# pvjosue/CWFA

Hardware: AMD Instinct MI355X
Metric: volumes/sec inverse-pass @512×512×96 fp32; NLL match vs ref (1/2/4/8 GPU) (higher is better)
Workload: dtype f32 (storage, accumulation, wavelets, couplings); convolution products on the bf16 matrix cores from an exact three-way bf16 split of both fp32 operands, six products per fp32 product: fp32-equivalent; plain-fp32-MFMA figure: fp32_mfma; 1 GPU; 512x512x96 volume, 4-scale CWFA (CAT blocks, 64 ch) + LRNN inverse, z=0, batch 1/GPU, random-init weights (BASELINE.json configs[2]); precision=split, parallelism=replicated x1 (independent volumes per GPU, no collective)

## Files before the change

cwfa_amd/_lib.py:

```python
import ctypes as C
import os

_HERE = os.path.dirname(os.path.abspath(__file__))
LIB_PATH = os.path.join(_HERE, "libcwfa_hip.so")

CLAMP = {"NONE": 0, "ATAN": 1, "TANH": 2, "SIGMOID": 3}
ACT = {None: 0, "none": 0, "elu": 1, "prelu": 2, "gelu": 3, "relu": 4}
CHAIN_MAX = 8

c_f32p = C.c_void_p
c_i64p = C.c_void_p
c_f64p = C.c_void_p


class AffineStage(C.Structure):
    _fields_ = [("s_raw", c_f32p), ("t", c_f32p), ("s_bs", C.c_int64), ("t_bs", C.c_int64), ("clamp_kind", C.c_int),
                ("clamp", C.c_float), ("pre_scale", C.c_float), ("t_neg_div_sqrt2", C.c_int), ("perm", c_i64p),
                ("perm_axis", C.c_int), ("gin", C.c_int)]


class Chain(C.Structure):
    _fields_ = [("n_stages", C.c_int), ("stage", AffineStage * CHAIN_MAX), ("src_c", C.c_void_p), ("src_h", C.c_void_p)]


class ChainGrads(C.Structure):
    _fields_ = [("ds", c_f32p * CHAIN_MAX), ("dt", c_f32p * CHAIN_MAX), ("ds_bs", C.c_int64 * CHAIN_MAX),
                ("dt_bs", C.c_int64 * CHAIN_MAX)]


class ConvOpts(C.Structure):
    _fields_ = [("bias", c_f32p), ("act", C.c_int), ("prelu_alpha", c_f32p), ("residual", c_f32p), ("res_bs", C.c_int64),
                ("act2", C.c_int), ("in_scale", c_f32p), ("in_shift", c_f32p), ("in_affine_bs", C.c_int), ("in_add", c_f32p),
                ("in_add_bs", C.c_int64), ("upshuffle2", C.c_int), ("in_blocked8", C.c_int), ("out_blocked8", C.c_int),
                ("in_cat", c_f32p), ("in_cat_bs", C.c_int64), ("in_cat_from", C.c_int), ("in_cat_c1", C.c_int), ("out_stats", c_f64p), ("prelu_per_channel", C.c_int)]


class Couple(C.Structure):
    _fields_ = [("x", c_f32p), ("y", c_f32p), ("x_bs", C.c_int64), ("y_bs", C.c_int64), ("n", C.c_int), ("clamp_kind", C.c_int),
                ("clamp", C.c_float), ("pre_scale", C.c_float), ("rev", C.c_int), ("logdet", c_f64p), ("in_blocked8", C.c_int)]


class EvalAffine(C.Structure):
    _fields_ = [("enabled", C.c_int), ("scale", C.c_float), ("std", C.c_float), ("mean", C.c_float)]


class EvalPost(C.Structure):
    _fields_ = [("normalize", C.c_int), ("threshold", C.c_int), ("norm_sub", C.c_float), ("norm_div", C.c_float),
                ("vol_min", C.c_float), ("lower", C.c_float), ("upper", C.c_float), ("clamp_value", C.c_float)]


EXTREMA_STRIDE = 12
SELECT_WORKSPACE_BYTES = 8448

i, i64, f, d, p = C.c_int, C.c_int64, C.c_float, C.c_double, C.c_void_p
SIGNATURES = {
    "cwfa_version": (i, []),
    "cwfa_last_error": (C.c_char_p, []),
    "cwfa_set_option": (i, [C.c_char_p, i]),
    "cwfa_haar1d_fwd_f32": (i, [p, p, p, i, i, i64, i64, i64, i64, p]),
    "cwfa_haar1d_inv_f32": (i, [p, p, p, i, i, i64, i64, i64, i64, p]),
    "cwfa_haar2d_fwd_f32": (i, [p, p, i, i, i, i, i, f, p]),
    "cwfa_haar2d_inv_f32": (i, [p, p, i, i, i, i, i, f, p]),
    "cwfa_haar3d_fwd_f32": (i, [p, p, i, i, i, i, i, f, i64, p]),
    "cwfa_haar3d_inv_f32": (i, [p, p, i, i, i, i, i, f, i64, p]),
    "cwfa_gather_f32": (i, [p, p, p, i, i, i, i, i, i64, i64, p]),
    "cwfa_affine_f32": (i, [p, p, C.POINTER(AffineStage), i, i, i, i, i, i64, i64, p, p, p]),
    "cwfa_channel_affine_f32": (i, [p, p, p, p, i, p, p, i, i, i64, i64, i64, p]),
# ... 101 lines not shown
```

cwfa_amd/csrc/conv2d.hip:

```cpp
#include "conv_internal.h"

#include <string.h>
#include <type_traits>

namespace {

template <int KS_, int CK_, int MT_, int NT_, int WM_, int WN_, int XV_ = 1>
struct Cfg {
    static constexpr int KS = KS_, CK = CK_, MT = MT_, NT = NT_, WM = WM_, WN = WN_;
    static constexpr int XV = XV_;
    static_assert(XV_ == 1 || (XV_ == 4 && KS_ == 1), "vector staging needs halo-free tiles");
    static constexpr int PAD = KS / 2;
    static constexpr int NTHREADS = 64 * WM * WN;
    static constexpr int CT = 32 * MT * WM;
    static constexpr int TR = NT * WN;
    static constexpr int TC = 32;
    static constexpr int XR = TR + KS - 1;
    static constexpr int XC = TC + KS - 1;
    static constexpr int XS = CK * XR * XC;
    static constexpr int XS_PAD = (XS + 3) & ~3;
    static constexpr int WS = KS * KS * CK * CT;
    static constexpr int XPT = (XS / XV + NTHREADS - 1) / NTHREADS;
    static constexpr int WPT = (WS / 4 + NTHREADS - 1) / NTHREADS;
    static constexpr int BUF = XS_PAD + WS;
// ... 539 lines not shown
            if constexpr (ALLOWED & (1u << EPI_NONE_BLK8)) return launch_epi<C, EPI_NONE_BLK8, PRO>(p, st);
            cwfa_set_error("cwfa_conv2d_f32: out_blocked8 is built for the 1x1 kernels with more than 32 output channels");
            return CWFA_E_SHAPE;
        default: break;
    }
    return launch_epi<C, EPI_GENERIC, PRO>(p, st);
}

template <class C, unsigned ALLOWED, unsigned ALLOWED_PRO>
int launch(const ConvParams& p, int epi, hipStream_t st) {
    if (p.o.in_scale || p.o.in_add) return launch_sel<C, ALLOWED_PRO, true>(p, epi, st);
    return launch_sel<C, ALLOWED, false>(p, epi, st);
}

}
int g_cwfa_split_xcd_map = 1;
int g_cwfa_split_rows16 = 1;
extern int g_cwfa_mip3_ablate;
namespace {

int fill_params(ConvParams& p, const char* name, const float* x, const float* w_packed, float* y, int B, int Cin, int H,
                int W, int Cout, int64_t x_bs, int64_t y_bs, const cwfa_conv_opts* opts) {
    CWFA_REQUIRE(B >= 0 && Cin > 0 && Cout > 0 && H >= 0 && W >= 0, CWFA_E_INVAL, "%s: bad size", name);
    if (B == 0 || H == 0 || W == 0) return 1;
    CWFA_REQUIRE(x && w_packed && y, CWFA_E_INVAL, "%s: null pointer", name);
    CWFA_REQUIRE((int64_t)Cin * H * W < (1ll << 30) && (int64_t)Cout * H * W * (p.o.upshuffle2 ? 1 : 1) < (1ll << 30), CWFA_E_SHAPE, "%s: C*H*W exceeds the 32-bit byte offsets of a tile (2^30 elements per image)", name);
    CWFA_REQUIRE(cwfa_aligned16(w_packed), CWFA_E_ALIGN, "%s: packed weights must be 16-byte aligned", name);
    p.x = x; p.wp = w_packed; p.y = y;
    p.B = B; p.Cin = Cin; p.H = H; p.W = W; p.Cout = Cout;
    p.x_bs = x_bs; p.y_bs = y_bs;
    p.products = g_cwfa_operand == CwfaOperand::split3 ? 6 : 1;
    if (opts) p.o = *opts;
    CWFA_REQUIRE(!(p.o.in_scale && !p.o.in_shift), CWFA_E_INVAL, "%s: in_scale without in_shift", name);
    CWFA_REQUIRE(p.o.act >= 0 && p.o.act <= CWFA_ACT_RELU && p.o.act2 >= 0 && p.o.act2 <= CWFA_ACT_RELU, CWFA_E_INVAL,
                 "%s: bad activation", name);
    CWFA_REQUIRE(!((p.o.act == CWFA_ACT_PRELU || p.o.act2 == CWFA_ACT_PRELU) && !p.o.prelu_alpha), CWFA_E_INVAL,
                 "%s: PReLU without prelu_alpha", name);
    return CWFA_OK;
}

typedef Cfg<1, 16, 2, 4, 4, 2> CS;
constexpr int CS_XB = 3 * 2 * 8 * 32 * 16, CS_WB = 3 * 2 * 256 * 16, CS_BUFB = CS_XB + CS_WB;

__device__ __forceinline__ void split3(float v, unsigned short (&o)[3]) {
    const __bf16 a1 = (__bf16)v;
    const float r1 = v - (float)a1;
    const __bf16 a2 = (__bf16)r1;
    const float r2 = r1 - (float)a2;
    const __bf16 a3 = (__bf16)r2;
    o[0] = __builtin_bit_cast(unsigned short, a1);
    o[1] = __builtin_bit_cast(unsigned short, a2);
    o[2] = __builtin_bit_cast(unsigned short, a3);
}

__device__ __forceinline__ unsigned short f16_bits(float v) { return __builtin_bit_cast(unsigned short, (_Float16)v); }

template <bool F16 = false>
__global__ __launch_bounds__(256) void split_input_kernel(const float* __restrict__ x, uint4* __restrict__ ws, int Cin, int CG2,
                                                          int64_t HW, int64_t x_bs, const float* __restrict__ sc,
                                                          const float* __restrict__ sh, int64_t aff_bs,
                                                          const float* __restrict__ add, int64_t add_bs) {
    const int64_t px = (int64_t)blockIdx.x * 256 + threadIdx.x;
    if (px >= HW) return;
    const int cg = blockIdx.y, b = blockIdx.z;
    unsigned short pc[3][8];
#pragma unroll
// ... 433 lines not shown
```

cwfa_amd/csrc/conv_split3x3.hip:

```cpp
#include "conv_internal.h"

extern int g_cwfa_split_xcd_map;
extern int g_cwfa_split_rows16;

namespace {

constexpr int TR = 8, TC = 32;

template <int KS, int RPW = 4>
struct XG {
    static constexpr int TRW = 2 * RPW, NT = 2 * RPW;
    static constexpr int PAD = KS / 2, XR = TRW + 2 * PAD, XC = TC + 2 * PAD, NTAP = KS * KS;
    static constexpr int EPK = XR * XC;
    static constexpr int KHB = KS == 7 ? 8512 : RPW == 8 ? 9792 : 5440;
    static constexpr int XPB = 2 * KHB;
    static constexpr int XB = 3 * XPB;
    static constexpr bool SPECIAL = KS == 3 && RPW == 4;
    static constexpr int NEK = SPECIAL ? 2 : 3;
    static_assert(EPK * 16 <= KHB && KHB % 256 == 64 && 2 * EPK <= 512 * NEK, "staging entry map");
    static_assert(!SPECIAL || (EPK > 256 && EPK <= 384), "3x3 staging entry map");
    static_assert(KS == 3 || RPW == 4, "7x7: 8-row tiles");
};

template <int MPW, int KS = 3, int RPW = 4, int WM = 4>
// ... 55 lines not shown

    constexpr int NEK = G::NEK;
    int ekh[NEK], eidx[NEK];
    bool fin[NEK];
    unsigned fo[NEK];
    if constexpr (SPECIAL) {
        ekh[0] = wave >> 2; eidx[0] = tid & 255; fin[0] = true;
        ekh[1] = (wave >> 1) & 1; eidx[1] = 256 + (tid & 127); fin[1] = wave < 4 && eidx[1] < EPK;
    } else {
#pragma unroll
        for (int k = 0; k < NEK; ++k) {
            const int e = tid + 512 * k;
            ekh[k] = e >= EPK;
            eidx[k] = e - ekh[k] * EPK;
            fin[k] = e < 2 * EPK;
        }
    }
    bool fok[NEK];
#pragma unroll
    for (int k = 0; k < NEK; ++k) {
        const int r = eidx[k] / XC, c = eidx[k] % XC;
        const int gr = row0 + r - PAD, gc = col0 + c - PAD;
        fok[k] = fin[k] && gr >= 0 && gr < p.H && gc >= 0 && gc < p.W;
        fo[k] = !fok[k] ? OOB : p.o.in_blocked8 ? (unsigned)((gr * p.W + gc) * 32) : (unsigned)((gr * p.W + gc) * 4);
        if constexpr (!SPECIAL) fo[k] = !fok[k] ? OOB : fo[k] + (unsigned)(ekh[k] * 8) * (unsigned)plane;
    }
    const int xbytes = p.Cin * plane;
    const auto rx = CWFA_RSRC(p.x + (int64_t)b * p.x_bs, xbytes);
    const auto ra = CWFA_RSRC(ADD ? p.o.in_add + (int64_t)b * p.o.in_add_bs : p.x, ADD ? xbytes : 0);
    const bool has_aff = p.o.in_scale != nullptr;
    typedef const float __attribute__((address_space(4))) cfloat;
    cfloat* sc = has_aff ? (cfloat*)(p.o.in_scale + (int64_t)b * p.o.in_affine_bs) : nullptr;
    cfloat* sh = has_aff ? (cfloat*)(p.o.in_shift + (int64_t)b * p.o.in_affine_bs) : nullptr;

    auto load_entry = [&](auto kc, float (&xv)[8], float (&av)[8], int chunk) {
        constexpr int k = decltype(kc)::value;
        const int ch0 = chunk * 16 + (SPECIAL ? ekh[k] * 8 : 0);
        if (KS == 3 && !ADD && p.o.in_blocked8) {
            const f32x4 lo4 = __builtin_bit_cast(f32x4, __builtin_amdgcn_raw_buffer_load_b128(rx, fo[k], ch0 * plane, 0));
            const f32x4 hi4 = __builtin_bit_cast(f32x4, __builtin_amdgcn_raw_buffer_load_b128(rx, fo[k], ch0 * plane + 16, 0));
#pragma unroll
            for (int j = 0; j < 4; ++j) {
                xv[j] = lo4[j];
                xv[4 + j] = hi4[j];
            }
            return;
        }
#pragma unroll
        for (int j = 0; j < 8; ++j) xv[j] = __builtin_bit_cast(float, __builtin_amdgcn_raw_buffer_load_b32(rx, fo[k], (ch0 + j) * plane, 0));
        if constexpr (ADD) {
#pragma unroll
            for (int j = 0; j < 8; ++j) av[j] = __builtin_bit_cast(float, __builtin_amdgcn_raw_buffer_load_b32(ra, fo[k], (ch0 + j) * plane, 0));
        }
    };
    auto store_entry = [&](auto kc, const float (&xv)[8], const float (&av)[8], int chunk, int buf) {
        constexpr int k = decltype(kc)::value;
        if (SPECIAL && k == 1 && !fin[1]) return;
        const int ch0 = chunk * 16 + ekh[k] * 8;
        bf16x8 pc[3];
        float scv[8], shv[8];
        if (has_aff) {
#pragma unroll
            for (int j = 0; j < 8; ++j) {
                const int ch = ch0 + j < p.Cin ? ch0 + j : p.Cin - 1;
                scv[j] = ch0 + j < p.Cin ? sc[ch] : 0.f;
                shv[j] = ch0 + j < p.Cin ? sh[ch] : 0.f;
            }
        }
#pragma unroll
        for (int j = 0; j < 8; ++j) {
            float v = xv[j];
            if (has_aff) v = fok[k] ? v * scv[j] + shv[j] : 0.f;
            if constexpr (ADD) v += av[j];
            __bf16 a1, a2 = (__bf16)0.f, a3 = (__bf16)0.f;
            cwfa_split3<SIX, F16>(v, a1, a2, a3);
            pc[0][j] = a1; pc[1][j] = a2; pc[2][j] = a3;
        }
        char* dst = lds + buf * XB + ekh[k] * KHB + eidx[k] * 16;
        if (SPECIAL || fin[k]) {
#pragma unroll
            for (int q = 0; q < NQ; ++q) *reinterpret_cast<bf16x8*>(dst + q * XPB) = pc[q];
        }
    };

    constexpr int NPC = (SIX ? WSL : WSL / 3) / 1024;
    const int64_t wtile = (int64_t)ct * p.nsteps * WSL;
    const char* wbase = reinterpret_cast<const char*>(p.wp) + wtile;
    const auto rw = CWFA_RSRC(wbase, p.nsteps * WSL);
    auto dma_w = [&](int slice, int slot) {
        cwfa_static_for<(NPC + 7) / 8>([&](auto ic_) {
            constexpr int i = decltype(ic_)::value;
            const int piece = i * 8 + wave;
            if (piece < NPC) {
                char* dst = lds + OFF_W + slot * WSL + piece * 1024;
                __builtin_amdgcn_raw_ptr_buffer_load_lds(rw, (lds_ptr)dst, 16, (unsigned)(lane * 16), slice * WSL + piece * 1024, 0, 0);
            }
        });
    };

    const int alane = OFF_W + (g * CT + wm * MPW * 16 + c16) * 16;
    const int blane = (g & 1) * KHB + (wn * RW * XC + c16) * 16;
    const bool sel = (g >> 1) != 0;

    f32x4 acc[MPW][NT];
#pragma unroll
    for (int mt = 0; mt < MPW; ++mt)
// ... 438 lines not shown

extern "C" int64_t cwfa_conv3x3_split_packed_bytes(int Cout, int Cin) {
    if (Cout <= 0 || Cin <= 0) return -1;
    const int ct = ct_of(Cout);
    return (int64_t)((Cout + ct - 1) / ct) * nsteps_of(Cin) * 3 * 4 * ct * 16;
}

extern "C" int cwfa_conv3x3_split_pack_f32(const float* w, void* packed, int Cout, int Cin, void* stream) {
    CWFA_REQUIRE(w && packed, CWFA_E_INVAL, "cwfa_conv3x3_split_pack_f32: null pointer");
    CWFA_REQUIRE(Cout > 0 && Cin > 0, CWFA_E_SHAPE, "cwfa_conv3x3_split_pack_f32: bad shape");
    CWFA_REQUIRE(cwfa_aligned16(packed), CWFA_E_ALIGN, "cwfa_conv3x3_split_pack_f32: packed image must be 16-byte aligned");
    pack_bank(w, packed, Cout, Cin, ct_of(Cout), 9, (hipStream_t)stream);
    CWFA_LAUNCH_CHECK("cwfa_conv3x3_split_pack_f32");
    return CWFA_OK;
}

extern "C" int cwfa_conv3x3_split_f32(const float* x, const void* w_packed, float* y, int B, int Cin, int H, int W, int Cout,
                                      int64_t x_bs, int64_t y_bs, const cwfa_conv_opts* opts, void* stream) {
    CWFA_REQUIRE(B >= 0 && Cin > 0 && Cout > 0 && H >= 0 && W >= 0, CWFA_E_INVAL, "cwfa_conv3x3_split_f32: bad size");
    if (B == 0 || H == 0 || W == 0) return CWFA_OK;
    CWFA_REQUIRE(x && w_packed && y, CWFA_E_INVAL, "cwfa_conv3x3_split_f32: null pointer");
    CWFA_REQUIRE(cwfa_aligned16(w_packed), CWFA_E_ALIGN, "cwfa_conv3x3_split_f32: packed weights must be 16-byte aligned");
    SParams p{};
    p.x = x; p.wp = w_packed; p.y = y;
    p.B = B; p.Cin = Cin; p.H = H; p.W = W; p.Cout = Cout; p.x_bs = x_bs; p.y_bs = y_bs;
    if (opts) p.o = *opts;
    CWFA_REQUIRE(!p.o.upshuffle2 && !p.o.in_cat, CWFA_E_SHAPE, "cwfa_conv3x3_split_f32: upshuffle2 / in_cat are 1x1 features");
    CWFA_REQUIRE(!p.o.in_blocked8 || (Cin % 8 == 0 && cwfa_aligned16(x) && (x_bs & 3) == 0 && !p.o.in_add), CWFA_E_ALIGN,
                 "cwfa_conv3x3_split_f32: blocked input needs Cin %% 8 == 0, 16-byte alignment and no added tensor");
    CWFA_REQUIRE(!p.o.out_blocked8 || (Cout % 8 == 0 && cwfa_aligned16(y) && (y_bs & 3) == 0 && !p.o.residual && p.o.act2 == CWFA_ACT_NONE &&
                                       (p.o.act == CWFA_ACT_NONE || p.o.act == CWFA_ACT_PRELU)),
                 CWFA_E_ALIGN, "cwfa_conv3x3_split_f32: blocked output needs Cout %% 8 == 0, 16-byte alignment and a bias / PReLU epilogue");
    CWFA_REQUIRE(!(p.o.in_scale && !p.o.in_shift), CWFA_E_INVAL, "cwfa_conv3x3_split_f32: in_scale without in_shift");
    CWFA_REQUIRE(!p.o.out_stats || (!p.o.out_blocked8 && !p.o.residual && p.o.act2 == CWFA_ACT_NONE &&
                                    (p.o.act == CWFA_ACT_NONE || p.o.act == CWFA_ACT_PRELU)),
                 CWFA_E_INVAL, "cwfa_conv3x3_split_f32: out_stats needs an NCHW output and a bias / PReLU epilogue");
    CWFA_REQUIRE(!((p.o.out_stats || p.o.out_blocked8) && p.o.in_add && p.o.act == CWFA_ACT_NONE), CWFA_E_INVAL,
                 "cwfa_conv3x3_split_f32: out_stats / out_blocked8 with in_add need a PReLU epilogue");
    CWFA_REQUIRE(p.o.act >= 0 && p.o.act <= CWFA_ACT_RELU && p.o.act2 >= 0 && p.o.act2 <= CWFA_ACT_RELU, CWFA_E_INVAL,
                 "cwfa_conv3x3_split_f32: bad activation");
    CWFA_REQUIRE(!((p.o.act == CWFA_ACT_PRELU || p.o.act2 == CWFA_ACT_PRELU) && !p.o.prelu_alpha), CWFA_E_INVAL,
                 "cwfa_conv3x3_split_f32: PReLU without prelu_alpha");
    p.nchunks = (Cin + 15) / 16;
    p.nsteps = nsteps_of(Cin);
    p.nrun = p.nsteps - ((p.nchunks & 1) ? 4 : 0);
    p.tiles_x = (W + TC - 1) / TC;
    const int mpw = mpw_of(Cout);
    CWFA_REQUIRE((int64_t)(Cin + 64) * H * W * 4 < (1ll << 31) && (int64_t)(Cout + 64 * mpw) * H * W * 4 < (1ll << 31) &&
                     (int64_t)(p.nsteps + 2) * 3 * 4 * 64 * mpw * 16 < (1ll << 31), CWFA_E_SHAPE,
                 "cwfa_conv3x3_split_f32: one sample's input / output / one cout tile's weights must stay below 2 GiB");
    CWFA_REQUIRE((int64_t)p.tiles_x * ((H + TR - 1) / TR) < (1ll << 31) && B <= 65535, CWFA_E_SHAPE, "cwfa_conv3x3_split_f32: grid too large");
    hipStream_t st = (hipStream_t)stream;
    const int wm = wm_of(Cout);
    if (wm != 4) {
        CWFA_REQUIRE(!p.o.in_scale && !p.o.in_add && !p.o.out_blocked8, CWFA_E_INVAL,
                     "cwfa_conv3x3_split_f32: banks with <= 48 or 65 .. 96 outputs take no load-side prologue and write NCHW");
        const bool plain = !p.o.residual && p.o.act2 == CWFA_ACT_NONE;
        const int epi = plain && p.o.act == CWFA_ACT_NONE ? 0 : plain && p.o.act == CWFA_ACT_PRELU ? 1 : 2;
#define CWFA_NARROW(M, W_)                                                                                                                   \
    do {                                                                                                                                     \
        if (epi == 0) return launch<M, false, CWFA_ACT_NONE, 3, 8, W_>(p, st);                                                               \
        if (epi == 1) return launch<M, false, CWFA_ACT_PRELU, 3, 8, W_>(p, st);                                                              \
        return launch<M, false, EPI_RUNTIME, 3, 8, W_>(p, st);                                                                               \
    } while (0)
        if (mpw == 3 && wm == 2) CWFA_NARROW(3, 2);
        if (mpw == 3) CWFA_NARROW(3, 1);
        if (mpw == 2) CWFA_NARROW(2, 1);
        CWFA_NARROW(1, 1);
#undef CWFA_NARROW
    }
    if (mpw == 4) return launch_epi<4>(p, st);
    if (mpw == 2) return launch_epi<2>(p, st);
    if (g_cwfa_split_rows16 && H > 8 && !p.o.in_scale && !p.o.in_add && !p.o.residual && p.o.act == CWFA_ACT_NONE && p.o.act2 == CWFA_ACT_NONE)
        return launch<2, false, CWFA_ACT_NONE, 3, 8, 2>(p, st);
    if (g_cwfa_split_rows16 && H > 8 && !p.o.in_scale && !p.o.in_add && !p.o.out_stats && !p.o.out_blocked8)
        return launch<2, false, EPI_RUNTIME, 3, 8, 2>(p, st);
    return launch_epi<1>(p, st);
}

extern "C" int64_t cwfa_conv7x7_split_packed_bytes(int Cout, int Cin) {
    if (Cout <= 0 || Cout > 64 || Cin <= 0) return -1;
    return (int64_t)nsteps_of(Cin, 49) * 3 * 4 * 64 * 16;
}

extern "C" int cwfa_conv7x7_split_pack_f32(const float* w, void* packed, int Cout, int Cin, void* stream) {
    CWFA_REQUIRE(w && packed, CWFA_E_INVAL, "cwfa_conv7x7_split_pack_f32: null pointer");
    CWFA_REQUIRE(Cout > 0 && Cout <= 64 && Cin > 0, CWFA_E_SHAPE, "cwfa_conv7x7_split_pack_f32: 1 <= Cout <= 64");
    CWFA_REQUIRE(cwfa_aligned16(packed), CWFA_E_ALIGN, "cwfa_conv7x7_split_pack_f32: packed image must be 16-byte aligned");
    pack_bank(w, packed, Cout, Cin, 64, 49, (hipStream_t)stream);
    CWFA_LAUNCH_CHECK("cwfa_conv7x7_split_pack_f32");
    return CWFA_OK;
}

extern "C" int cwfa_conv7x7_split_f32(const float* x, const void* w_packed, float* y, int B, int Cin, int H, int W, int Cout,
                                      int64_t x_bs, int64_t y_bs, const cwfa_conv_opts* opts, void* stream) {
    CWFA_REQUIRE(B >= 0 && Cin > 0 && Cout > 0 && Cout <= 64 && H >= 0 && W >= 0, CWFA_E_INVAL, "cwfa_conv7x7_split_f32: bad size (Cout <= 64)");
    if (B == 0 || H == 0 || W == 0) return CWFA_OK;
    CWFA_REQUIRE(x && w_packed && y, CWFA_E_INVAL, "cwfa_conv7x7_split_f32: null pointer");
    CWFA_REQUIRE(cwfa_aligned16(w_packed), CWFA_E_ALIGN, "cwfa_conv7x7_split_f32: packed weights must be 16-byte aligned");
    SParams p{};
    p.x = x; p.wp = w_packed; p.y = y;
    p.B = B; p.Cin = Cin; p.H = H; p.W = W; p.Cout = Cout; p.x_bs = x_bs; p.y_bs = y_bs;
    if (opts) p.o = *opts;
    CWFA_REQUIRE(!p.o.upshuffle2 && !p.o.in_cat && !p.o.in_scale && !p.o.in_add && !p.o.in_blocked8 && !p.o.out_blocked8 && !p.o.residual && !p.o.out_stats &&
                     p.o.act == CWFA_ACT_NONE && p.o.act2 == CWFA_ACT_NONE,
                 CWFA_E_INVAL, "cwfa_conv7x7_split_f32: bias-only epilogue, no load-side prologue, NCHW maps");
    p.nchunks = (Cin + 15) / 16;
    p.nsteps = nsteps_of(Cin, 49);
    p.nrun = p.nsteps;
    p.tiles_x = (W + TC - 1) / TC;
    CWFA_REQUIRE((int64_t)(Cin + 64) * H * W * 4 < (1ll << 31) && (int64_t)(Cout + 64) * H * W * 4 < (1ll << 31), CWFA_E_SHAPE,
                 "cwfa_conv7x7_split_f32: one sample's input / output must stay below 2 GiB");
    CWFA_REQUIRE((int64_t)p.tiles_x * ((H + TR - 1) / TR) < (1ll << 31) && B <= 65535, CWFA_E_SHAPE, "cwfa_conv7x7_split_f32: grid too large");
    hipStream_t st = (hipStream_t)stream;
    return launch<2, false, CWFA_ACT_NONE, 7, 4, 2>(p, st);
}
```

cwfa_amd/ops.py:

```python
import ctypes as C

import torch

from . import _lib
from ._lib import AffineStage, Chain, ConvOpts, check

__all__ = ["haar1d", "haar2d", "gather", "affine", "channel_affine", "chain_inv", "chain_fwd", "pack_conv_weight",
           "conv2d", "conv2d_wgrad", "elu_bwd", "set_precision", "gelu_add", "gelu_bwd", "layernorm_bwd", "attention_bwd", "plane_affine", "bn_bwd_stats", "bn_act_bwd", "maxpool2_bwd", "chain_bwd", "chain_inv_bwd", "prelu_bwd", "conv3d_1k1_backward", "pack_1x1_panel", "pack_split_layer_weight", "subnet_layer", "conv3d_1k1", "channel_stats", "bn_fold", "bn_running_update", "maxpool", "sample_stats", "layernorm_apply",
           "attention_combine", "scale_channels", "axpby", "stage"]


def _stream():
    return C.c_void_p(torch.cuda.current_stream().cuda_stream)


def _p(t):
    return None if t is None else C.c_void_p(t.data_ptr())


def _dev(t, name="tensor"):
    if not torch.is_tensor(t):
        raise TypeError(f"{name}: expected a torch.Tensor, got {type(t)}")
    if not t.is_cuda:
        raise RuntimeError(f"{name}: cwfa_amd runs on MI355X only -- got a {t.device} tensor (no CPU fallback exists)")
# ... 343 lines not shown
        return PackedConv(packed, cout, cin, ks, transposed, w._version, w.data_ptr(), split=True)
    if not direct and SPLIT_7X7 and _split_bf16 >= 2 and ks == 7 and cout <= 64 and cin >= 32:
        packed = torch.empty(L.cwfa_conv7x7_split_packed_bytes(cout, cin), dtype=torch.uint8, device=w.device)
        check(L.cwfa_conv7x7_split_pack_f32(_p(w), _p(packed), cout, cin, _stream()), "conv7x7_split_pack")
        return PackedConv(packed, cout, cin, ks, transposed, w._version, w.data_ptr(), split=True)
    n = L.cwfa_conv2d_packed_floats(cout, cin, ks)
    if n <= 0:
        raise ValueError(f"unsupported filter bank {tuple(w.shape)}")
    packed = torch.empty(n, dtype=torch.float32, device=w.device)
    check(L.cwfa_conv2d_pack_f32(_p(w), _p(packed), cout, cin, ks, int(transposed), _stream()), "conv2d_pack")
    return PackedConv(packed, cout, cin, ks, transposed, w._version, w.data_ptr())


def pack_conv_weight_cat(w, c1):
    w = _dev(w, "weight").detach()
    cout, cin, ks, kw = w.shape
    if ks != 1 or kw != 1 or cout > 64 or not (0 < c1 < cin):
        raise ValueError(f"pack_conv_weight_cat: a 1x1 bank with <= 64 outputs and 0 < c1 < Cin is needed, got {tuple(w.shape)}, c1 = {c1}")
    start = (c1 + 15) // 16 * 16
    wz = torch.zeros((cout, start + cin - c1, 1, 1), dtype=torch.float32, device=w.device)
    wz[:, :c1] = w[:, :c1]
    wz[:, start:] = w[:, c1:]
    pc = pack_conv_weight(wz)
    pc.version, pc.src_ptr = w._version, w.data_ptr()
    pc.cat_c1, pc.cat_from = c1, start
    return pc


def conv_writes_stats(pc, act=None, residual=None, act2=None, out_blocked=False, in_add=False):
    return bool(pc.split and pc.ks == 3 and act in (None, "prelu") and residual is None and act2 is None and not out_blocked
                and not (in_add and act is None))


def conv2d(x, pc, bias=None, act=None, prelu_alpha=None, residual=None, act2=None, in_scale=None, in_shift=None,
           in_add=None, out=None, in_blocked=False, out_blocked=False, cat=None, out_stats=None):
    L = _lib.lib()
    x, xbs = planes(x, "x")
    B, Cin, H, W = x.shape
    o = ConvOpts()
    keep = [x]
    if cat is not None:
        cat, cbs = planes(cat, "cat")
        c1 = getattr(pc, "cat_c1", None)
        if c1 is None or Cin != c1 or tuple(cat.shape) != (B, pc.cin - pc.cat_from, H, W) or in_scale is not None or in_add is not None:
            raise ValueError("conv2d: `cat` needs a bank from pack_conv_weight_cat for exactly these two inputs, and no load-side prologue")
        o.in_cat, o.in_cat_bs, o.in_cat_from, o.in_cat_c1 = cat.data_ptr(), cbs, pc.cat_from, c1
        keep.append(cat)
        Cin = pc.cin
    if Cin != pc.cin:
        raise ValueError(f"conv2d: input has {Cin} channels, filter bank expects {pc.cin}")
    up = bool(pc.transposed)
    oshape = (B, pc.cout // 4, 2 * H, 2 * W) if up else (B, pc.cout, H, W)
    if out is None:
        out = torch.empty(oshape, dtype=torch.float32, device=x.device)
        ybs = oshape[1] * oshape[2] * oshape[3]
    else:
        if tuple(out.shape) != oshape:
            raise ValueError(f"conv2d: out has shape {tuple(out.shape)}, expected {oshape}")
        out_c, ybs = planes(out, "out")
        if out_c.data_ptr() != out.data_ptr():
            raise ValueError("conv2d: `out` must have contiguous planes")
    if bias is not None:
        o.bias = _dev(bias, "bias").data_ptr()
    o.act, o.act2 = _lib.ACT[act], _lib.ACT[act2]
    if prelu_alpha is not None:
        prelu_alpha = _dev(prelu_alpha, "prelu_alpha")
        o.prelu_alpha = prelu_alpha.data_ptr()
        if prelu_alpha.numel() != 1:
            if prelu_alpha.numel() != pc.cout or not prelu_alpha.is_contiguous() or not (pc.split and pc.ks == 3):
                raise ValueError("conv2d: per-channel PReLU slopes need [Cout] contiguous values and the split-bf16 3x3 kernel")
            o.prelu_per_channel = 1
    elif "prelu" in (act, act2):
        raise ValueError("conv2d: PReLU needs prelu_alpha")
    if residual is not None:
        residual, rbs = planes(residual, "residual")
        if tuple(residual.shape) != oshape:
            raise ValueError(f"conv2d: residual {tuple(residual.shape)} != output {oshape}")
        o.residual, o.res_bs = residual.data_ptr(), rbs
        keep.append(residual)
    if in_scale is not None:
        o.in_scale, o.in_shift = _dev(in_scale).data_ptr(), _dev(in_shift).data_ptr()
        if in_scale.numel() not in (Cin, B * Cin) or in_shift.numel() != in_scale.numel():
            raise ValueError("conv2d: in_scale / in_shift must be [Cin] or [B,Cin]")
        o.in_affine_bs = Cin if (in_scale.numel() == B * Cin and B > 1) else 0
    if in_add is not None:
        in_add, abs_ = planes(in_add, "in_add")
        if tuple(in_add.shape) != tuple(x.shape):
            raise ValueError("conv2d: in_add shape mismatch")
        o.in_add, o.in_add_bs = in_add.data_ptr(), abs_
        keep.append(in_add)
    o.upshuffle2 = int(up)
    if in_blocked:
        if not (pc.split and pc.ks == 3):
            raise ValueError("conv2d: channel-blocked input is read by the split-bf16 3x3 kernel only")
        o.in_blocked8 = 1
    if out_blocked:
        ok3 = (pc.split and pc.ks == 3 and pc.cout % 8 == 0 and residual is None and act2 is None and act in (None, "prelu")
               and not split3x3_narrow(pc.cout) and not (in_add is not None and act is None))
        ok1 = not pc.split and pc.ks == 1 and pc.cout >= 33 and pc.cout % 8 == 0 and not up
        if not (ok3 or ok1):
            raise ValueError("conv2d: channel-blocked output is written by the split-bf16 3x3 kernel (bias / PReLU) and by the "
                             "direct 1x1 kernel with 40..64 output channels only")
        o.out_blocked8 = 1
    if out_stats is not None:
        if not conv_writes_stats(pc, act, residual, act2, out_blocked, in_add is not None):
            raise ValueError("conv2d: out_stats needs the split-bf16 3x3 kernel with an NCHW output and a bias / PReLU epilogue")
        if out_stats.dtype != torch.float64 or out_stats.numel() != 2 * pc.cout or not out_stats.is_cuda:
            raise ValueError("conv2d: out_stats must be a float64 [2*Cout] tensor on the HIP device")
        o.out_stats = out_stats.data_ptr()
    rec = conv_event_sink
    if rec is not None:
        key = (pc.ks, Cin, pc.cout, H, W, B, "%s|%s|%s|%s|%s" % ("pro" if (in_scale is not None or in_add is not None) else "",
                                                                 act or "", "res" if residual is not None else "", act2 or "",
                                                                 ("up" if up else "") + ("+split" if pc.split else "")),
               in_add is not None)
        if rec.want(key):
            e0, e1 = torch.cuda.Event(enable_timing=True), torch.cuda.Event(enable_timing=True)
            e0.record()
    if pc.split and pc.ks == 7:
        if act or act2 or residual is not None or in_scale is not None or in_add is not None:
            raise ValueError("conv2d: the split-bf16 7x7 kernel has a bias-only epilogue and no load-side prologue")
        check(L.cwfa_conv7x7_split_f32(_p(x), _p(pc.packed), _p(out), B, Cin, H, W, pc.cout, xbs, ybs, C.byref(o), _stream()),
              "conv7x7_split")
# ... 58 lines not shown
def conv3x3_couple(u, pc_bias, x, out, clamp_kind, clamp, pre_scale, rev, logdet=None, in_blocked=False):
    L = _lib.lib()
    pc, br = pc_bias
    u, ubs = planes(u, "u")
    B, Cin, H, W = u.shape
    n = pc.cout // 2
    if Cin != pc.cin:
        raise ValueError(f"conv3x3_couple: input has {Cin} channels, filter bank expects {pc.cin}")
    x2, xbs = planes(x, "x")
    o2, obs = planes(out, "out")
    if tuple(x.shape) != (B, n, H, W) or tuple(out.shape) != (B, n, H, W) or o2.data_ptr() != out.data_ptr():
        raise ValueError("conv3x3_couple: x / out must be [B,n,H,W] views with contiguous planes")
    cp = _lib.Couple()
    cp.x, cp.y, cp.x_bs, cp.y_bs, cp.n = x2.data_ptr(), out.data_ptr(), xbs, obs, n
    cp.clamp_kind, cp.clamp, cp.pre_scale, cp.rev = _lib.CLAMP[clamp_kind], float(clamp), float(pre_scale), int(bool(rev))
    if logdet is not None:
        cp.logdet = logdet.data_ptr()
    cp.in_blocked8 = int(bool(in_blocked))
    rec = conv_event_sink
    if rec is not None:
        key = (3, Cin, pc.cout, H, W, B, "||||couple+split", False)
        if rec.want(key):
            e0, e1 = torch.cuda.Event(enable_timing=True), torch.cuda.Event(enable_timing=True)
            e0.record()
    check(L.cwfa_conv3x3_split_couple_f32(_p(u), _p(pc.packed), _p(br), B, Cin, H, W, ubs, C.byref(cp), _stream()),
          "conv3x3_split_couple")
    if rec is not None and rec.want(key):
        e1.record()
        rec.add(key, e0, e1)
    return out


BLOCKED_MAPS = True
SPLIT_7X7 = True
VIRTUAL_CAT = True
COUPLE_EPILOGUE = True


def couple_fused():
    return COUPLE_EPILOGUE and _split_bf16 >= 2


def split3x3_narrow(cout):
    return cout <= 48 or 64 < cout <= 96


SPLIT_3X3_MIN_COUT = 1
SPLIT_3X3_NARROW_MAX = 16
conv_event_sink = None


def pack_1x1_panel(w):
    L = _lib.lib()
    w = _dev(w, "weight").detach().contiguous()
    if tuple(w.shape) != (64, 64, 1, 1):
        raise ValueError("pack_1x1_panel: the fused layer kernel is specialised for 64 channels")
    panel = torch.empty(4096, dtype=torch.float32, device=w.device)
    check(L.cwfa_subnet_pack1x1_f32(_p(w), _p(panel), _stream()), "subnet_pack1x1")
    return PackedConv(panel, 64, 64, 1, False, w._version, w.data_ptr())


def pack_split_layer_weight(w3, w1):
    L = _lib.lib()
    w3 = _dev(w3, "weight").detach().contiguous()
    w1 = _dev(w1, "weight").detach().contiguous()
    if tuple(w3.shape) != (64, 64, 3, 3) or tuple(w1.shape) != (64, 64, 1, 1):
# ... 709 lines not shown
```

cwfa_amd/unet.py:

```python
import torch
from torch import nn

from . import ops
from .amp import amp_entry

__all__ = ["UNet", "UNetConvBlock", "UNetUpBlock"]


_MATERIALIZE_UP = False
_MATERIALIZE = True


class _Packed:

    def __init__(self):
        self._c = {}

    def get(self, conv, transposed=False):
        w = conv.weight
        pc = self._c.get(id(conv))
        if pc is None or pc.version != w._version or pc.src_ptr != w.data_ptr() or pc.epoch != ops.pack_epoch():
            pc = self._c[id(conv)] = ops.pack_conv_weight(w, transposed=transposed)
        return pc

# ... 81 lines not shown
                 activation=nn.LeakyReLU):
        super().__init__()
        if stride != 1 or kernel_size != 3 or not padding:
            raise NotImplementedError("cwfa_amd UNetConvBlock: 3x3, stride 1, padded convolutions only")
        block = [nn.Conv2d(in_size, out_size, kernel_size=kernel_size, stride=stride, padding=int(padding), bias=use_bias),
                 activation()]
        if batch_norm:
            block.append(nn.BatchNorm2d(out_size))
        block += [nn.Conv2d(out_size, out_size, kernel_size=kernel_size, stride=1, padding=int(padding), bias=use_bias),
                  activation()]
        if batch_norm:
            block.append(nn.BatchNorm2d(out_size))
        self.block = nn.Sequential(*block)
        self.batch_norm = batch_norm
        self._packed = _Packed()

    def _layers(self):
        mods = list(self.block)
        step = 3 if self.batch_norm else 2
        return [(mods[i], mods[i + 1], mods[i + 2] if self.batch_norm else None) for i in (0, step)]

    @staticmethod
    def _act(a):
        if isinstance(a, nn.PReLU):
            if a.weight.numel() != 1:
                raise NotImplementedError("per-channel PReLU")
            return "prelu", a.weight
        if isinstance(a, nn.ELU):
            return "elu", None
        if isinstance(a, nn.ReLU):
            return "relu", None
        raise NotImplementedError(f"activation {type(a).__name__} has no HIP epilogue")

    def run(self, x, in_affine=None, in_add=None, out_mask=None):
        aff = in_affine
        layers = self._layers()
        packs = [self._packed.get(conv) for conv, _, _ in layers]
        for li, (conv, act, bn) in enumerate(layers):
            kind, alpha = self._act(act)
            sc, sh = aff if aff is not None else (None, None)
            add = in_add if li == 0 else None
            if (_MATERIALIZE and ops._split_bf16 < 2 and (sc is not None or add is not None)
                    and (x.shape[2] * x.shape[3]) % 4 == 0):
                x = ops.plane_affine(x, sc, sh, add=add)
                sc = sh = add = None
            st = None
            if (STATS_IN_EPILOGUE and bn is not None and _bn_batch_stats(bn)
                    and ops.conv_writes_stats(packs[li], kind, in_add=add is not None)):
                st = _bn_stats_buffer(bn, x.device)
            x = ops.conv2d(x, packs[li], bias=conv.bias, act=kind, prelu_alpha=alpha, in_scale=sc,
                           in_shift=sh, in_add=add, out_stats=st)
            last = li == len(layers) - 1
            m = out_mask if last else None
            if bn is not None:
                aff = _bn_affine(bn, x, m, stats=st)
            elif m is not None:
                aff = _drop_affine(x.shape[1], m)
            else:
                aff = None
        return x, aff

    @amp_entry
    def forward(self, x):
        y, aff = self.run(x)
        if aff is None:
            return y
        return ops.channel_affine(y, aff[0], aff[1])


class UNetUpBlock(nn.Module):

    def __init__(self, in_size, out_size, up_mode, padding, batch_norm, use_bias=False, skip_conn=True,
                 activation=nn.Softplus):
        super().__init__()
        self.skip_conn = skip_conn
        if up_mode != 'upconv':
            raise NotImplementedError("cwfa_amd UNetUpBlock: up_mode='upconv' only (what the LRNN uses, networks.py:532)")
        self.up = nn.ConvTranspose2d(in_size, out_size, kernel_size=2, stride=2, bias=use_bias)
        in_size = out_size if not skip_conn else in_size // 2
        self.conv_block = UNetConvBlock(in_size, out_size, padding, batch_norm, use_bias=use_bias, activation=activation)
        self._packed = _Packed()

    @staticmethod
    def center_crop(layer, target_size):
        _, _, h, w = layer.size()
        dy, dx = (h - target_size[0]) // 2, (w - target_size[1]) // 2
        return layer[:, :, dy:(dy + target_size[0]), dx:(dx + target_size[1])]

    def run(self, x, bridge, in_affine=None, out_mask=None):
        sc, sh = in_affine if in_affine is not None else (None, None)
        if _MATERIALIZE_UP and ops._split_bf16 < 1 and sc is not None and (x.shape[2] * x.shape[3]) % 4 == 0:
            x = ops.plane_affine(x, sc, sh)
            sc = sh = None
        up = ops.conv2d(x, self._packed.get(self.up, transposed=True), bias=self.up.bias, in_scale=sc, in_shift=sh)
        add = self.center_crop(bridge, up.shape[2:]) if self.skip_conn else None
        return self.conv_block.run(up, in_add=add, out_mask=out_mask)

    @amp_entry
    def forward(self, x, bridge):
        y, aff = self.run(x, bridge)
        return y if aff is None else ops.channel_affine(y, aff[0], aff[1])


class UNet(nn.Module):

    def __init__(self, in_channels=1, n_classes=2, depth=5, wf=6, padding=True, batch_norm=True, up_mode='upsample',
                 drop_out=0, use_bias=False, skip_conn=False, activation=nn.PReLU):
        super().__init__()
        assert up_mode in ('upconv', 'upsample')
        self.padding, self.depth, self.skip_conn, self.drop_out = padding, depth, skip_conn, drop_out
        prev = in_channels
        self.down_path = nn.ModuleList()
        for i in range(depth):
            self.down_path.append(UNetConvBlock(prev, 2 ** (wf + i), padding, batch_norm, use_bias=use_bias,
                                                activation=activation))
            prev = 2 ** (wf + i)
        self.up_path = nn.ModuleList()
        for i in reversed(range(depth - 1)):
            self.up_path.append(UNetUpBlock(prev, 2 ** (wf + i), up_mode, padding, batch_norm, use_bias=use_bias,
                                            skip_conn=skip_conn, activation=activation))
            prev = 2 ** (wf + i)
        self.last = nn.Sequential(nn.Conv2d(prev, n_classes, kernel_size=1, bias=use_bias), activation())
        self._packed = _Packed()

    @amp_entry
    def forward(self, x, store_activations=False, in_affine=None):
        if store_activations:
            raise NotImplementedError("store_activations is a debugging aid of the reference, not on the hot path")
        B, dev = x.shape[0], x.device
        skips, aff = [], in_affine
        n_draw = 0
        if self.drop_out:
            n_draw = B * (sum(d.block[0].out_channels for d in list(self.down_path)[:-1]) +
                          sum(u.conv_block.block[0].out_channels for u in self.up_path))
        pool = _DrawPool(n_draw, dev)
        for i, down in enumerate(self.down_path):
            x, aff = down.run(x, in_affine=aff)
            if i != len(self.down_path) - 1:
                sc, sh = aff if aff is not None else (None, None)
                x, full = ops.maxpool(x, x.shape[-1] // 2, x.shape[-1] // 2, sc, sh, want_full=True)
                skips.append(full)
                m = _drop(self.drop_out, B, x.shape[1], dev, pool)
                aff = _drop_affine(x.shape[1], m) if m is not None else None
        for i, up in enumerate(self.up_path):
            m = _drop(self.drop_out, B, up.conv_block.block[0].out_channels, dev, pool)
            x, aff = up.run(x, skips[-i - 1], in_affine=aff, out_mask=m)
        kind, alpha = UNetConvBlock._act(self.last[1])
        sc, sh = aff if aff is not None else (None, None)
        return ops.conv2d(x, self._packed.get(self.last[0]), bias=self.last[0].bias, act=kind, prelu_alpha=alpha,
                          in_scale=sc, in_shift=sh)
```

include/cwfa_hip.h:

```cpp
#ifndef CWFA_HIP_H
#define CWFA_HIP_H

#include <stdint.h>

#ifdef __cplusplus
extern "C" {
#endif

#define CWFA_VERSION 100

enum {
    CWFA_OK = 0,
    CWFA_E_INVAL = -1,
    CWFA_E_SHAPE = -2,
    CWFA_E_ALIGN = -3,
    CWFA_E_HIP = -4
};

enum { CWFA_CLAMP_NONE = 0, CWFA_CLAMP_ATAN = 1, CWFA_CLAMP_TANH = 2, CWFA_CLAMP_SIGMOID = 3 };

enum { CWFA_ACT_NONE = 0, CWFA_ACT_ELU = 1, CWFA_ACT_PRELU = 2, CWFA_ACT_GELU = 3, CWFA_ACT_RELU = 4 };

int cwfa_version(void);
const char* cwfa_last_error(void);
// ... 51 lines not shown
} cwfa_chain;

int cwfa_chain_inv_f32(const float* z, const float* low, float* x, const cwfa_chain* ch, int B, int C, int H, int W,
                       int64_t z_bs, int64_t low_bs, int64_t x_bs, double* logdet, void* stream);

int cwfa_chain_fwd_f32(const float* x, float* low, float* z, const cwfa_chain* ch, const int64_t* final_perm,
                       int B, int C, int H, int W, int64_t x_bs, int64_t low_bs, int64_t z_bs,
                       double* logdet, double* sumsq, void* stream);


int64_t cwfa_conv2d_packed_floats(int Cout, int Cin, int ks);
int cwfa_conv2d_pack_f32(const float* w, float* packed, int Cout, int Cin, int ks, int transposed, void* stream);

typedef struct {
    const float* bias;
    int act;
    const float* prelu_alpha;
    const float* residual;
    int64_t res_bs;
    int act2;
    const float* in_scale;
    const float* in_shift;
    int in_affine_bs;
    const float* in_add;
    int64_t in_add_bs;
    int upshuffle2;
    int in_blocked8;
    int out_blocked8;
    const float* in_cat;
    int64_t in_cat_bs;
    int in_cat_from, in_cat_c1;
    double* out_stats;
    int prelu_per_channel;
} cwfa_conv_opts;

int cwfa_conv2d_f32(const float* x, const float* w_packed, float* y, int B, int Cin, int H, int W, int Cout, int ks,
                    int64_t x_bs, int64_t y_bs, const cwfa_conv_opts* opts, void* stream);

int cwfa_subnet_pack1x1_f32(const float* w, float* panel, void* stream);
int cwfa_subnet_layer_f32(const float* x, const float* w3_packed, const float* b3, const float* w1_panel, const float* b1,
                          float* y, int B, int H, int W, int64_t x_bs, int64_t y_bs, void* stream);
int cwfa_subnet_layer_tape_f32(const float* x, const float* w3_packed, const float* b3, const float* w1_panel, const float* b1,
                               float* y, float* hidden, int B, int H, int W, int64_t x_bs, int64_t y_bs, int64_t hidden_bs,
                               void* stream);

int cwfa_conv3d_1k1_f32(const float* x, const float* w1, const float* b1, const float* alpha, const float* w2,
                        const float* b2, float* y, int B, int D, int H, int W, int K, void* stream);
int cwfa_conv3d_1k1_split_f32(const float* x, const float* w1, const float* b1, const float* alpha, const float* w2,
                              const float* b2, float* y, int B, int D, int H, int W, int K, void* stream);


int cwfa_channel_stats_f32(const float* x, double* stats, int B, int C, int64_t HW, int64_t x_bs, void* stream);
int cwfa_bn_fold_f32(const double* stats, double count, const float* running_mean, const float* running_var,
                     const float* weight, const float* bias, float eps, const float* mask_bc, int B, float* scale,
                     float* shift, int C, void* stream);
int cwfa_bn_finish_f32(double* stats, double count, float* running_mean, float* running_var, long long* num_batches_tracked,
                       float momentum, int update_running, const float* weight, const float* bias, float eps, const float* mask_bc,
                       const float* mask_u, float drop_p, float keep_scale, int B, float* scale, float* shift, int C, int zero_stats,
                       void* stream);
int cwfa_bn_running_update_f32(const double* stats, double count, float momentum, float* running_mean, float* running_var,
                               long long* num_batches_tracked, int C, void* stream);
int cwfa_maxpool_f32(const float* x, float* y, float* full, const float* scale, const float* shift, int B, int C,
                     int H, int W, int Ho, int Wo, void* stream);
int cwfa_sample_stats_f32(const float* x, double* stats, int B, int64_t CHW, void* stream);
int cwfa_layernorm_apply_f32(const float* x, const double* stats, const float* w, const float* b, float eps,
                             float* y, int B, int64_t CHW, void* stream);
// ... 134 lines not shown
```

Before: 52.44 volumes/s.

## Defer UNet skip-connection batchnorm affine into split 3x3 conv add-load

Instead of having maxpool write out a fully normalized copy of each down-path activation for the skip connection, the UNet keeps the raw pre-affine map plus its scale/shift. The first 3x3 split-bf16 conv of the matching up block then applies that per-channel affine to the in_add operand while loading it. The aim is to drop one full-resolution activation write and its later reread per skip level. In exchange, the conv staging path does extra per-channel scalar loads and FMAs, the raw skip tensors stay alive longer, and narrow tilings fall back to a separate channel_affine pass.

Result: no change. 52.51 volumes/s (median of 6 runs) (+0.1%).

```diff
diff --git a/cwfa_amd/_lib.py b/cwfa_amd/_lib.py
--- a/cwfa_amd/_lib.py
+++ b/cwfa_amd/_lib.py
@@ -32,7 +32,8 @@
     _fields_ = [("bias", c_f32p), ("act", C.c_int), ("prelu_alpha", c_f32p), ("residual", c_f32p), ("res_bs", C.c_int64),
                 ("act2", C.c_int), ("in_scale", c_f32p), ("in_shift", c_f32p), ("in_affine_bs", C.c_int), ("in_add", c_f32p),
                 ("in_add_bs", C.c_int64), ("upshuffle2", C.c_int), ("in_blocked8", C.c_int), ("out_blocked8", C.c_int),
-                ("in_cat", c_f32p), ("in_cat_bs", C.c_int64), ("in_cat_from", C.c_int), ("in_cat_c1", C.c_int), ("out_stats", c_f64p), ("prelu_per_channel", C.c_int)]
+                ("in_cat", c_f32p), ("in_cat_bs", C.c_int64), ("in_cat_from", C.c_int), ("in_cat_c1", C.c_int), ("out_stats", c_f64p), ("prelu_per_channel", C.c_int),
+                ("in_add_scale", c_f32p), ("in_add_shift", c_f32p), ("in_add_affine_bs", C.c_int)]
 
 
 class Couple(C.Structure):
diff --git a/cwfa_amd/csrc/conv2d.hip b/cwfa_amd/csrc/conv2d.hip
--- a/cwfa_amd/csrc/conv2d.hip
+++ b/cwfa_amd/csrc/conv2d.hip
@@ -595,6 +595,7 @@
     p.products = g_cwfa_operand == CwfaOperand::split3 ? 6 : 1;
     if (opts) p.o = *opts;
     CWFA_REQUIRE(!(p.o.in_scale && !p.o.in_shift), CWFA_E_INVAL, "%s: in_scale without in_shift", name);
+    CWFA_REQUIRE(!p.o.in_add_scale && !p.o.in_add_shift, CWFA_E_INVAL, "%s: in_add_scale / in_add_shift are features of cwfa_conv3x3_split_f32", name);
     CWFA_REQUIRE(p.o.act >= 0 && p.o.act <= CWFA_ACT_RELU && p.o.act2 >= 0 && p.o.act2 <= CWFA_ACT_RELU, CWFA_E_INVAL,
                  "%s: bad activation", name);
     CWFA_REQUIRE(!((p.o.act == CWFA_ACT_PRELU || p.o.act2 == CWFA_ACT_PRELU) && !p.o.prelu_alpha), CWFA_E_INVAL,
diff --git a/cwfa_amd/csrc/conv_split3x3.hip b/cwfa_amd/csrc/conv_split3x3.hip
--- a/cwfa_amd/csrc/conv_split3x3.hip
+++ b/cwfa_amd/csrc/conv_split3x3.hip
@@ -111,6 +111,7 @@
     typedef const float __attribute__((address_space(4))) cfloat;
     cfloat* sc = has_aff ? (cfloat*)(p.o.in_scale + (int64_t)b * p.o.in_affine_bs) : nullptr;
     cfloat* sh = has_aff ? (cfloat*)(p.o.in_shift + (int64_t)b * p.o.in_affine_bs) : nullptr;
+    const bool has_aaf = ADD && p.o.in_add_scale != nullptr;
 
     auto load_entry = [&](auto kc, float (&xv)[8], float (&av)[8], int chunk) {
         constexpr int k = decltype(kc)::value;
@@ -137,6 +138,25 @@
         if (SPECIAL && k == 1 && !fin[1]) return;
         const int ch0 = chunk * 16 + ekh[k] * 8;
         bf16x8 pc[3];
+        float adv[8];
+        if constexpr (ADD) {
+#pragma unroll
+            for (int j = 0; j < 8; ++j) adv[j] = av[j];
+            if (has_aaf) {
+                cfloat* asc = (cfloat*)(p.o.in_add_scale + (int64_t)b * p.o.in_add_affine_bs);
+                cfloat* ash = (cfloat*)(p.o.in_add_shift + (int64_t)b * p.o.in_add_affine_bs);
+                float tsc[8], tsh[8];
+#pragma unroll
+                for (int j = 0; j < 8; ++j) {
+                    const int ch = ch0 + j < p.Cin ? ch0 + j : p.Cin - 1;
+                    tsc[j] = ch0 + j < p.Cin ? asc[ch] : 0.f;
+                    tsh[j] = ch0 + j < p.Cin ? ash[ch] : 0.f;
+                }
+#pragma unroll
+                for (int j = 0; j < 8; ++j) adv[j] = fok[k] ? adv[j] * tsc[j] + tsh[j] : 0.f;
+                CWFA_FENCE();
+            }
+        }
         float scv[8], shv[8];
         if (has_aff) {
 #pragma unroll
@@ -150,7 +170,7 @@
         for (int j = 0; j < 8; ++j) {
             float v = xv[j];
             if (has_aff) v = fok[k] ? v * scv[j] + shv[j] : 0.f;
-            if constexpr (ADD) v += av[j];
+            if constexpr (ADD) v += adv[j];
             __bf16 a1, a2 = (__bf16)0.f, a3 = (__bf16)0.f;
             cwfa_split3<SIX, F16>(v, a1, a2, a3);
             pc[0][j] = a1; pc[1][j] = a2; pc[2][j] = a3;
@@ -655,6 +675,8 @@
                                        (p.o.act == CWFA_ACT_NONE || p.o.act == CWFA_ACT_PRELU)),
                  CWFA_E_ALIGN, "cwfa_conv3x3_split_f32: blocked output needs Cout %% 8 == 0, 16-byte alignment and a bias / PReLU epilogue");
     CWFA_REQUIRE(!(p.o.in_scale && !p.o.in_shift), CWFA_E_INVAL, "cwfa_conv3x3_split_f32: in_scale without in_shift");
+    CWFA_REQUIRE(!p.o.in_add_scale == !p.o.in_add_shift && !(p.o.in_add_scale && !p.o.in_add), CWFA_E_INVAL,
+                 "cwfa_conv3x3_split_f32: in_add_scale / in_add_shift come together and need in_add");
     CWFA_REQUIRE(!p.o.out_stats || (!p.o.out_blocked8 && !p.o.residual && p.o.act2 == CWFA_ACT_NONE &&
                                     (p.o.act == CWFA_ACT_NONE || p.o.act == CWFA_ACT_PRELU)),
                  CWFA_E_INVAL, "cwfa_conv3x3_split_f32: out_stats needs an NCHW output and a bias / PReLU epilogue");
@@ -676,7 +698,7 @@
     hipStream_t st = (hipStream_t)stream;
     const int wm = wm_of(Cout);
     if (wm != 4) {
-        CWFA_REQUIRE(!p.o.in_scale && !p.o.in_add && !p.o.out_blocked8, CWFA_E_INVAL,
+        CWFA_REQUIRE(!p.o.in_scale && !p.o.in_add && !p.o.in_add_scale && !p.o.out_blocked8, CWFA_E_INVAL,
                      "cwfa_conv3x3_split_f32: banks with <= 48 or 65 .. 96 outputs take no load-side prologue and write NCHW");
         const bool plain = !p.o.residual && p.o.act2 == CWFA_ACT_NONE;
         const int epi = plain && p.o.act == CWFA_ACT_NONE ? 0 : plain && p.o.act == CWFA_ACT_PRELU ? 1 : 2;
@@ -725,7 +747,7 @@
     p.x = x; p.wp = w_packed; p.y = y;
     p.B = B; p.Cin = Cin; p.H = H; p.W = W; p.Cout = Cout; p.x_bs = x_bs; p.y_bs = y_bs;
     if (opts) p.o = *opts;
-    CWFA_REQUIRE(!p.o.upshuffle2 && !p.o.in_cat && !p.o.in_scale && !p.o.in_add && !p.o.in_blocked8 && !p.o.out_blocked8 && !p.o.residual && !p.o.out_stats &&
+    CWFA_REQUIRE(!p.o.upshuffle2 && !p.o.in_cat && !p.o.in_scale && !p.o.in_add && !p.o.in_add_scale && !p.o.in_add_shift && !p.o.in_blocked8 && !p.o.out_blocked8 && !p.o.residual && !p.o.out_stats &&
                      p.o.act == CWFA_ACT_NONE && p.o.act2 == CWFA_ACT_NONE,
                  CWFA_E_INVAL, "cwfa_conv7x7_split_f32: bias-only epilogue, no load-side prologue, NCHW maps");
     p.nchunks = (Cin + 15) / 16;
diff --git a/cwfa_amd/ops.py b/cwfa_amd/ops.py
--- a/cwfa_amd/ops.py
+++ b/cwfa_amd/ops.py
@@ -399,8 +399,12 @@
                 and not (in_add and act is None))
 
 
+def conv_takes_add_affine(pc):
+    return bool(SKIP_AFFINE_ON_LOAD and pc.split and pc.ks == 3 and not split3x3_narrow(pc.cout))
+
+
 def conv2d(x, pc, bias=None, act=None, prelu_alpha=None, residual=None, act2=None, in_scale=None, in_shift=None,
-           in_add=None, out=None, in_blocked=False, out_blocked=False, cat=None, out_stats=None):
+           in_add=None, out=None, in_blocked=False, out_blocked=False, cat=None, out_stats=None, add_scale=None, add_shift=None):
     L = _lib.lib()
     x, xbs = planes(x, "x")
     B, Cin, H, W = x.shape
@@ -456,6 +460,13 @@
             raise ValueError("conv2d: in_add shape mismatch")
         o.in_add, o.in_add_bs = in_add.data_ptr(), abs_
         keep.append(in_add)
+    if add_scale is not None or add_shift is not None:
+        if in_add is None or add_scale is None or add_shift is None or not conv_takes_add_affine(pc):
+            raise ValueError("conv2d: add_scale / add_shift come together, with in_add, on the split-bf16 3x3 kernel's wide tilings only")
+        if add_scale.numel() not in (Cin, B * Cin) or add_shift.numel() != add_scale.numel():
+            raise ValueError("conv2d: add_scale / add_shift must be [Cin] or [B,Cin]")
+        o.in_add_scale, o.in_add_shift = _dev(add_scale).data_ptr(), _dev(add_shift).data_ptr()
+        o.in_add_affine_bs = Cin if (add_scale.numel() == B * Cin and B > 1) else 0
     o.upshuffle2 = int(up)
     if in_blocked:
         if not (pc.split and pc.ks == 3):
@@ -580,6 +591,7 @@
 
 
 BLOCKED_MAPS = True
+SKIP_AFFINE_ON_LOAD = True
 SPLIT_7X7 = True
 VIRTUAL_CAT = True
 COUPLE_EPILOGUE = True
diff --git a/cwfa_amd/unet.py b/cwfa_amd/unet.py
--- a/cwfa_amd/unet.py
+++ b/cwfa_amd/unet.py
@@ -137,10 +137,13 @@
             return "relu", None
         raise NotImplementedError(f"activation {type(a).__name__} has no HIP epilogue")
 
-    def run(self, x, in_affine=None, in_add=None, out_mask=None):
+    def run(self, x, in_affine=None, in_add=None, out_mask=None, add_affine=None):
         aff = in_affine
         layers = self._layers()
         packs = [self._packed.get(conv) for conv, _, _ in layers]
+        if add_affine is not None and not ops.conv_takes_add_affine(packs[0]):
+            in_add, add_affine = ops.channel_affine(in_add, add_affine[0], add_affine[1]), None
+        asc, ash = add_affine if add_affine is not None else (None, None)
         for li, (conv, act, bn) in enumerate(layers):
             kind, alpha = self._act(act)
             sc, sh = aff if aff is not None else (None, None)
@@ -154,7 +157,8 @@
                     and ops.conv_writes_stats(packs[li], kind, in_add=add is not None)):
                 st = _bn_stats_buffer(bn, x.device)
             x = ops.conv2d(x, packs[li], bias=conv.bias, act=kind, prelu_alpha=alpha, in_scale=sc,
-                           in_shift=sh, in_add=add, out_stats=st)
+                           in_shift=sh, in_add=add, out_stats=st, add_scale=asc if li == 0 else None,
+                           add_shift=ash if li == 0 else None)
             last = li == len(layers) - 1
             m = out_mask if last else None
             if bn is not None:
@@ -192,14 +196,14 @@
         dy, dx = (h - target_size[0]) // 2, (w - target_size[1]) // 2
         return layer[:, :, dy:(dy + target_size[0]), dx:(dx + target_size[1])]
 
-    def run(self, x, bridge, in_affine=None, out_mask=None):
+    def run(self, x, bridge, in_affine=None, out_mask=None, bridge_affine=None):
         sc, sh = in_affine if in_affine is not None else (None, None)
         if _MATERIALIZE_UP and ops._split_bf16 < 1 and sc is not None and (x.shape[2] * x.shape[3]) % 4 == 0:
             x = ops.plane_affine(x, sc, sh)
             sc = sh = None
         up = ops.conv2d(x, self._packed.get(self.up, transposed=True), bias=self.up.bias, in_scale=sc, in_shift=sh)
         add = self.center_crop(bridge, up.shape[2:]) if self.skip_conn else None
-        return self.conv_block.run(up, in_add=add, out_mask=out_mask)
+        return self.conv_block.run(up, in_add=add, out_mask=out_mask, add_affine=bridge_affine if self.skip_conn else None)
 
     @amp_entry
     def forward(self, x, bridge):
@@ -234,6 +238,7 @@
             raise NotImplementedError("store_activations is a debugging aid of the reference, not on the hot path")
         B, dev = x.shape[0], x.device
         skips, aff = [], in_affine
+        raw_skip = self.skip_conn and ops.SKIP_AFFINE_ON_LOAD and ops._split_bf16 >= 2
         n_draw = 0
         if self.drop_out:
             n_draw = B * (sum(d.block[0].out_channels for d in list(self.down_path)[:-1]) +
@@ -243,13 +248,18 @@
             x, aff = down.run(x, in_affine=aff)
             if i != len(self.down_path) - 1:
                 sc, sh = aff if aff is not None else (None, None)
-                x, full = ops.maxpool(x, x.shape[-1] // 2, x.shape[-1] // 2, sc, sh, want_full=True)
-                skips.append(full)
+                if raw_skip:
+                    skips.append((x, aff))
+                    x = ops.maxpool(x, x.shape[-1] // 2, x.shape[-1] // 2, sc, sh, want_full=False)
+                else:
+                    x, full = ops.maxpool(x, x.shape[-1] // 2, x.shape[-1] // 2, sc, sh, want_full=True)
+                    skips.append((full, None))
                 m = _drop(self.drop_out, B, x.shape[1], dev, pool)
                 aff = _drop_affine(x.shape[1], m) if m is not None else None
         for i, up in enumerate(self.up_path):
             m = _drop(self.drop_out, B, up.conv_block.block[0].out_channels, dev, pool)
-            x, aff = up.run(x, skips[-i - 1], in_affine=aff, out_mask=m)
+            bridge, baff = skips[-i - 1]
+            x, aff = up.run(x, bridge, in_affine=aff, out_mask=m, bridge_affine=baff)
         kind, alpha = UNetConvBlock._act(self.last[1])
         sc, sh = aff if aff is not None else (None, None)
         return ops.conv2d(x, self._packed.get(self.last[0]), bias=self.last[0].bias, act=kind, prelu_alpha=alpha,
diff --git a/include/cwfa_hip.h b/include/cwfa_hip.h
--- a/include/cwfa_hip.h
+++ b/include/cwfa_hip.h
@@ -107,6 +107,9 @@
     int in_cat_from, in_cat_c1;
     double* out_stats;
     int prelu_per_channel;
+    const float* in_add_scale;
+    const float* in_add_shift;
+    int in_add_affine_bs;
 } cwfa_conv_opts;
 
 int cwfa_conv2d_f32(const float* x, const float* w_packed, float* y, int B, int Cin, int H, int W, int Cout, int ks,
```
